# zixunh/vipe

Measured on AMD Instinct MI355X. Metric: dense-BA+flow update iters/s, 512x384 48-KF graph, higher is better.
Workload: dtype f16 (correlation, GRU; fp32 accumulate) + f32 geometry/BA (fp64 reduced system)

## Files before the change

### include/vipe_amd.h

```cpp
#ifndef VIPE_AMD_H
#define VIPE_AMD_H

#include <stdint.h>

#ifdef __cplusplus
extern "C" {
#endif

#define VIPE_F16 0
#define VIPE_F32 1
#define VIPE_F64 2
#define VIPE_U8 3

#define VIPE_OK 0
#define VIPE_EINVAL (-1)
#define VIPE_ENOSPACE (-2)
#define VIPE_EUNSUPPORTED (-3)

#define VIPE_PYRAMID_REFERENCE 0
#define VIPE_PYRAMID_BLOCKED 1

#define VIPE_CAM_PINHOLE 0
#define VIPE_CAM_MEI 1
#define VIPE_CAM_PANORAMA 2
// ... 237 lines not shown
int vipe_conv_packed_dims(int Cout, int Cin, int KH, int KW, int* cout_pad, int* cin_pad, int* k_pad);

#define VIPE_CONV_PARTIAL 6
#define VIPE_CONV_HEADS_FUSED 7
#define VIPE_CONV_ACCINIT_F32 0x100
int vipe_conv2d_fused(const void* d_x0, int x0_ctot, int x0_coff, const void* d_x1, int x1_ctot, int x1_coff,
                      int split, const void* d_w_packed, const float* d_bias, const float* d_extra, int extra_stride,
                      int extra_off, void* d_y, int y_ctot, int y_coff, void* d_y2, int y2_ctot, int y2_coff,
                      const void* d_net, int net_ctot, int net_coff, const void* d_z, float* d_fout,
                      const void* d_accinit, int ai_ctot, int ai_coff, int B, int H, int W, int Cin, int Cout, int KH,
                      int KW, int act, int mode, void* stream);

int vipe_heads_fused_ok(int H, int W);
int vipe_heads_border_floats(int E, int H, int W, int64_t* n_floats);
int vipe_heads_finish(float* d_dw, const float* d_border, const float* d_bias, int E, int H, int W, void* stream);

typedef struct {
  const void *corr0_w, *corr2_w, *flow0_w, *flow2_w, *gw_w, *zr_w, *q_w, *zr_s_w, *q_s_w, *heads0_w, *heads2_w, *agg2_w, *eta_w;
  const void *zr_n_w, *zr_x_w;
  const float *corr0_b, *corr2_b, *flow0_b, *flow2_b, *gw_b, *zr_b, *q_b, *heads0_b, *heads2_b, *agg2_b, *eta_b;
  const float* glo_wT;
  const float* glo_b;
  const void *agg1_w, *heads_dw_w;
  const float *agg1_b, *heads_dw_b;
  const void* heads2_frag;
} vipe_update_weights;
typedef struct {
  int E, H, W, n_src;
  const void* levels[4];
  const float* coords;
// ... 4 lines not shown
  const void* net;
  void* net_out;
  void* xbuf;
  const void* pgate;
  void *c1, *f1, *zb, *rnet;
  void* hbuf;
  float* dw;
  float *glo, *extra;
  const int *order, *rowptr;
  void *agg, *a2;
  float* eta;
  void* side_stream;
  float* pzr;
  int gate_state;
  float* hborder;
} vipe_update_buffers;
int vipe_update_operator(const vipe_update_weights* weights, const vipe_update_buffers* buffers, void* stream);

int vipe_update_gate_state(const vipe_update_weights* weights, const vipe_update_buffers* buffers, const void* d_net,
                           int parts, void* stream);
typedef struct {
  const vipe_update_weights* weights;
  const vipe_update_buffers* buffers;
  const void* net;
  const int* bounds;
  int n_bounds;
} vipe_gate_state_job;
int vipe_update_gate_state_piece(void* user, int piece, int n_pieces, void* stream);

int vipe_glo_context(const float* d_glo_sum, const float* d_wT, const float* d_bias, float* d_extra, int E, int hw,
// ... 93 lines not shown
```

### vipe_amd/csrc/common.cuh

```cuda
#pragma once
#include <hip/hip_runtime.h>
#include <hip/hip_fp16.h>
#include <stdint.h>

#include <atomic>
#include <mutex>

#include "../../include/vipe_amd.h"

#define VIPE_EXPORT extern "C" __attribute__((visibility("default")))

#define VIPE_CHECK_ARG(cond) \
  do {                       \
    if (!(cond)) return VIPE_EINVAL; \
  } while (0)

static inline int vipe_launch_status() {
  hipError_t e = hipGetLastError();
  return e == hipSuccess ? VIPE_OK : (int)e;
}

template <typename F>
static inline void vipe_once_per_device(std::atomic<uint64_t>& done, F&& fn) {
  int d = 0;
  (void)hipGetDevice(&d);
  const uint64_t bit = 1ull << (d & 63);
  if (done.load(std::memory_order_acquire) & bit) return;
  static std::mutex mu;
  std::lock_guard<std::mutex> lock(mu);
  if (done.load(std::memory_order_relaxed) & bit) return;
  fn();
  done.fetch_or(bit, std::memory_order_release);
}

static inline hipStream_t as_stream(void* s) { return (hipStream_t)s; }

constexpr int WAVE = 64;

template <typename T>
__device__ __forceinline__ T wave_sum(T v) {
#pragma unroll
  for (int o = 32; o > 0; o >>= 1) v += __shfl_xor(v, o, WAVE);
  return v;
}

__device__ __forceinline__ float wave_sum_to_lane63(float v) {
#define VIPE_DPP_ADD(ctrl, rmask)                                                                          \
  v += __builtin_bit_cast(float, __builtin_amdgcn_update_dpp(0, __builtin_bit_cast(int, v), ctrl, rmask, 0xf, true))
  VIPE_DPP_ADD(0xB1, 0xf);
  VIPE_DPP_ADD(0x4E, 0xf);
  VIPE_DPP_ADD(0x141, 0xf);
// ... 22 lines not shown
```

### vipe_amd/csrc/conv_mfma.hip

```cpp
#include <stdlib.h>

#include <type_traits>

#include "common.cuh"
#include "conv_call.cuh"

namespace {

typedef _Float16 half8 __attribute__((ext_vector_type(8)));
typedef _Float16 half4 __attribute__((ext_vector_type(4)));
typedef float float16v __attribute__((ext_vector_type(16)));
typedef float float4v __attribute__((ext_vector_type(4)));

struct ConvArgs {
  const half_t* x0; int x0_ctot, x0_coff;
  const half_t* x1; int x1_ctot, x1_coff;
  int split;
  const half_t* w;
  const float* bias;
  const float* extra;
  int extra_stride, extra_off;
  half_t* y; int y_ctot, y_coff;
  int B, H, W, Cin, Cin_pad, Cout, Cout_pad, KH, KW, nsteps;
  int act, epi;
// ... 1144 lines not shown
  VIPE_CHECK_ARG(d_w_oihw && d_w_packed);
  VIPE_CHECK_ARG(src_dtype == VIPE_F16 || src_dtype == VIPE_F32);
  int cp, cinp, kp;
  if (vipe_conv_packed_dims(Cout, Cin, KH, KW, &cp, &cinp, &kp) != VIPE_OK) return VIPE_EINVAL;
  VIPE_CHECK_ARG(Cin == 4 || Cin % 8 == 0);
  const int64_t total = (int64_t)kp * cp;
  pack_weights_kernel<<<(int)std::min<int64_t>((total + 255) / 256, 4096), 256, 0, as_stream(stream)>>>(
      d_w_oihw, (half_t*)d_w_packed, Cout, Cin, KH, KW, cp, cinp, kp, src_dtype == VIPE_F32, Cin == 4);
  return vipe_launch_status();
}

}

namespace {

__global__ __launch_bounds__(256) void heads_finish_kernel(float* __restrict__ dw, const float* __restrict__ border,
                                                           const float* __restrict__ bias, int64_t M, int H, int W) {
  const int64_t m = (int64_t)blockIdx.x * 256 + threadIdx.x;
  if (m >= M) return;
  const int x = (int)(m % W), y = (int)((m / W) % H), e = (int)(m / ((int64_t)W * H));
  const int xsegs = W / HALO_TW, ysegs = H / HALO_TH;
  const int ty = y / HALO_TH, tx = x / HALO_TW, py = y % HALO_TH, px = x % HALO_TW;
  const int tile = (e * ysegs + ty) * xsegs + tx;
  float4 s = reinterpret_cast<const float4*>(dw)[m];
  auto add = [&](int t, int bi) {
    const float4 v = reinterpret_cast<const float4*>(border)[(int64_t)t * HB_N + bi];
    s.x += v.x; s.y += v.y; s.z += v.z; s.w += v.w;
  };
  const bool up = py == 0 && ty > 0, down = py == HALO_TH - 1 && ty < ysegs - 1;
  const bool left = px == 0 && tx > 0, right = px == HALO_TW - 1 && tx < xsegs - 1;
  if (up) add(tile - xsegs, hb_index(HALO_TH, px));
  if (down) add(tile + xsegs, hb_index(-1, px));
  if (left) add(tile - 1, hb_index(py, HALO_TW));
  if (right) add(tile + 1, hb_index(py, -1));
  if (up && left) add(tile - xsegs - 1, hb_index(HALO_TH, HALO_TW));
  if (up && right) add(tile - xsegs + 1, hb_index(HALO_TH, -1));
  if (down && left) add(tile + xsegs - 1, hb_index(-1, HALO_TW));
  if (down && right) add(tile + xsegs + 1, hb_index(-1, -1));
  const float4 b = *reinterpret_cast<const float4*>(bias);
  const float v0 = s.x + b.x, v1 = s.y + b.y, v2 = s.z + b.z, v3 = s.w + b.w;
  reinterpret_cast<float4*>(dw)[m] = make_float4((float)(half_t)v0, (float)(half_t)v1, (float)(half_t)act_apply(v2, VIPE_ACT_SIGMOID),
                                                 (float)(half_t)act_apply(v3, VIPE_ACT_SIGMOID));
}

template <typename K>
void allow_lds(K kernel, std::atomic<uint64_t>& seen, size_t bytes) {
  vipe_once_per_device(seen, [&] { (void)hipFuncSetAttribute((const void*)kernel, hipFuncAttributeMaxDynamicSharedMemorySize, (int)bytes); });
}
constexpr size_t MAX_LDS = 160 * 1024;

bool flat_geometry(ConvArgs& a, int pad) {
  a.f_wp = a.W + pad;
  a.f_hwp = a.H * a.f_wp;
  a.f_tiles = (a.f_hwp + 255) / 256;
  a.f_magic = (unsigned)(((1ull << 32) + (unsigned)a.f_wp - 1) / (unsigned)a.f_wp);
  const int rows = 256 + 2 * a.f_wp + 2;
  a.f_pieces = (rows + 15) / 16;
// ... 209 lines not shown
VIPE_EXPORT int vipe_heads_border_floats(int E, int H, int W, int64_t* n) {
  VIPE_CHECK_ARG(n && E >= 0 && H > 0 && W > 0 && H % HALO_TH == 0 && W % HALO_TW == 0);
  *n = (int64_t)E * (H / HALO_TH) * (W / HALO_TW) * HB_N * 4;
  return VIPE_OK;
}

VIPE_EXPORT int vipe_heads_finish(float* d_dw, const float* d_border, const float* d_bias, int E, int H, int W, void* stream) {
  VIPE_CHECK_ARG(E >= 0 && H > 0 && W > 0 && H % HALO_TH == 0 && W % HALO_TW == 0);
  if (E == 0) return VIPE_OK;
  VIPE_CHECK_ARG(d_dw && d_border && d_bias);
  const int64_t M = (int64_t)E * H * W;
  heads_finish_kernel<<<(unsigned)((M + 255) / 256), 256, 0, as_stream(stream)>>>(d_dw, d_border, d_bias, M, H, W);
  return vipe_launch_status();
}

}
```

### vipe_amd/csrc/corr_lookup.hip

```cpp
#include <algorithm>
#include <type_traits>

#include "common.cuh"
#include "corr_layout.cuh"

namespace {

template <typename T>
struct Acc;

template <>
struct Acc<half_t> {
  using reg = float;
  static __device__ __forceinline__ reg load(const half_t* p) { return (float)*p; }
  static __device__ __forceinline__ reg weight(float w) {
    asm volatile("" : "+v"(w));
    return (float)(half_t)w;
  }
  static __device__ __forceinline__ reg madd(reg acc, reg s, reg w) {
    float prod = (float)(half_t)(s * w);
    return (float)(half_t)(acc + prod);
  }
  static __device__ __forceinline__ half_t store(reg v) { return (half_t)v; }
};
// ... 517 lines not shown
VIPE_EXPORT int vipe_corr_pyramid_lookup(const void* const* h_levels, const float* d_coords, void* d_out, int B,
                                         int h1, int w1, int h2, int w2, int num_levels, int radius, int dtype,
                                         void* stream) {
  return pyramid_lookup_impl(h_levels, d_coords, d_out, B, h1, w1, h2, w2, num_levels, radius, dtype, 0, stream);
}

VIPE_EXPORT int vipe_corr_pyramid_lookup_nhwc(const void* const* h_levels, const float* d_coords, void* d_out, int B,
                                              int h1, int w1, int h2, int w2, int num_levels, int radius, int dtype,
                                              int channel_stride, void* stream) {
  const int rd = 2 * radius + 1;
  VIPE_CHECK_ARG(channel_stride >= num_levels * rd * rd);
  return pyramid_lookup_impl(h_levels, d_coords, d_out, B, h1, w1, h2, w2, num_levels, radius, dtype, channel_stride,
                             stream);
}

static int device_compute_units() {
  static std::atomic<int> cus[64];
  int d = 0;
  (void)hipGetDevice(&d);
  int n = cus[d & 63].load(std::memory_order_relaxed);
  if (n > 0) return n;
  if (hipDeviceGetAttribute(&n, hipDeviceAttributeMultiprocessorCount, d) != hipSuccess || n <= 0) return 0;
  cus[d & 63].store(n, std::memory_order_relaxed);
  return n;
}

VIPE_EXPORT int vipe_corr_lookup_conv1x1(const void* const* h_levels, const float* d_coords, const void* d_w_packed,
                                         const float* d_bias, void* d_out, int out_ctot, int out_coff, int B, int h1,
                                         int w1, int h2, int w2, int Cout, int act, const int* d_slots, int layout,
                                         void* stream) {
  return vipe_corr_lookup_conv1x1_ex(h_levels, d_coords, d_w_packed, d_bias, d_out, out_ctot, out_coff, B, h1, w1, h2, w2,
                                     Cout, act, d_slots, layout, stream, 0, 0);
}

VIPE_EXPORT int vipe_corr_lookup_conv1x1_ex(const void* const* h_levels, const float* d_coords, const void* d_w_packed,
                                            const float* d_bias, void* d_out, int out_ctot, int out_coff, int B, int h1,
                                            int w1, int h2, int w2, int Cout, int act, const int* d_slots, int layout,
                                            void* stream, int max_workgroups, int share_cu) {
  VIPE_CHECK_ARG(B >= 0 && h1 > 0 && w1 > 0 && h2 > 0 && w2 > 0 && max_workgroups >= 0);
  if (B == 0) return VIPE_OK;
  VIPE_CHECK_ARG(h_levels && d_coords && d_w_packed && d_bias && d_out);
  VIPE_CHECK_ARG(act == VIPE_ACT_NONE || act == VIPE_ACT_RELU);
  VIPE_CHECK_ARG(out_ctot % 8 == 0 && out_coff % 8 == 0 && out_coff + Cout <= out_ctot);
  VIPE_CHECK_ARG(layout == VIPE_PYRAMID_REFERENCE || layout == VIPE_PYRAMID_BLOCKED);
  if (Cout != 128 || (h2 >> 3) < 1 || (w2 >> 3) < 1) return VIPE_EUNSUPPORTED;
  if (layout == VIPE_PYRAMID_REFERENCE && ((w2 >> 3) & 7) != 0) return VIPE_EUNSUPPORTED;
  if (layout == VIPE_PYRAMID_BLOCKED) VIPE_CHECK_ARG(h1 == h2 && w1 == w2);
  LevelPtrs lv;
  for (int i = 0; i < 4; ++i) {
    VIPE_CHECK_ARG(h_levels[i]);
    lv.p[i] = h_levels[i];
  }
  const int64_t ngroups = (int64_t)B * ((h1 * w1 + LKC_PX - 1) / LKC_PX);
  VIPE_CHECK_ARG(ngroups < (1 << 30));
  const int cus = device_compute_units();
  if (cus <= 0) return VIPE_EINVAL;
  int64_t blocks = std::min<int64_t>(ngroups, share_cu ? cus : 2 * cus);
  if (max_workgroups > 0) blocks = std::min<int64_t>(blocks, max_workgroups);
  const size_t lds = share_cu ? LKC_LDS_SHARED_CU : LKC_LDS;
  auto launch = [&](auto blk) {
    auto* kernel = corr_lookup_conv_kernel<decltype(blk)::value>;
    static std::atomic<uint64_t> seen{0};
    vipe_once_per_device(seen, [&] { (void)hipFuncSetAttribute((const void*)kernel, hipFuncAttributeMaxDynamicSharedMemorySize, LKC_LDS_SHARED_CU); });
    kernel<<<(int)blocks, LKC_THREADS, lds, as_stream(stream)>>>(lv, d_coords, (const half_t*)d_w_packed, d_bias, (half_t*)d_out,
                                                                 out_ctot, out_coff, h1, w1, h2, w2, B, 128, act, d_slots);
  };
  if (layout == VIPE_PYRAMID_BLOCKED) launch(std::true_type{});
  else launch(std::false_type{});
  return vipe_launch_status();
}
// ... 1 lines not shown
```

### vipe_amd/csrc/misc.hip

```cpp
#include "common.cuh"

VIPE_EXPORT const char* vipe_amd_version(void) { return "vipe_amd 0.1 (gfx950, hipcc)"; }
VIPE_EXPORT int vipe_amd_abi_version(void) { return 4; }
```

### vipe_amd/csrc/update_op.hip

```cpp
#include "common.cuh"
#include "conv_call.cuh"

namespace {

__global__ __launch_bounds__(384) void glo_gemm_kernel(const float* __restrict__ glo, const float* __restrict__ wT ,
                                                       const float* __restrict__ b, float* __restrict__ extra, float inv_hw) {
  __shared__ float g[128];
  const int e = blockIdx.x, t = threadIdx.x;
  if (t < 128) g[t] = glo[(int64_t)e * 128 + t] * inv_hw;
  __syncthreads();
  float acc = b[t];
#pragma unroll 8
  for (int k = 0; k < 128; ++k) acc = __builtin_fmaf(g[k], wT[k * 384 + t], acc);
  extra[(int64_t)e * 384 + t] = acc;
}

__global__ __launch_bounds__(256) void update_finish_kernel(const float* __restrict__ coords1, const float* __restrict__ dw,
                                                            const unsigned char* __restrict__ mask, float* __restrict__ target,
                                                            float* __restrict__ weight, const float* __restrict__ eta,
                                                            const int64_t* __restrict__ du, float* __restrict__ damping,
                                                            int64_t n_px, int64_t n_eta, int P) {
  const int64_t i = (int64_t)blockIdx.x * 256 + threadIdx.x;
  if (i < n_px) {
    const float2 c = reinterpret_cast<const float2*>(coords1)[i];
// ... 104 lines not shown
  auto agg_chain = [&](hipStream_t st) -> int {
    if (b->n_src <= 0) return VIPE_OK;
    VIPE_CHECK_ARG(b->order && b->rowptr && b->agg && b->a2 && b->eta);
    const Grid gs = {b->n_src, H, W};
    RUN(vipe_segment_mean_nhwc_f16(b->hbuf, 384, 256, b->order, b->rowptr, b->agg, b->n_src, (int64_t)H * W, 128, st));
    RUN(relu_conv(gs, {b->agg, 128, 0}, 128, wt->agg2_w, wt->agg2_b, 128, 3, {b->a2, 128, 0}, st));
    ConvCall c = conv(gs, {b->a2, 128, 0}, 128, wt->eta_w, wt->eta_b, 1, 3);
    c.epi = EPI_ETA; c.fout = b->eta;
    return vipe_conv_run(c, st);
  };
  auto heads2 = [&](hipStream_t st) -> int {
    ConvCall c = conv(g, {b->hbuf, 384, 0}, 256, wt->heads2_w, wt->heads2_b, 4, 3);
    c.epi = EPI_HEADS; c.fout = b->dw;
    return vipe_conv_run(c, st);
  };
  if (by_consumer && two_tails) {
    RUN(heads0(wt->agg1_w, wt->agg1_b, 256, 128));
    VIPE_CHECK_ARG(fork(2));
    RUN(agg_chain(side));
    if (wt->heads2_frag && b->hborder && vipe_heads_fused_ok(H, W)) {
      ConvCall c = conv(g, {b->net_out, 128, 0}, 128, wt->heads_dw_w, wt->heads_dw_b, 256, 3);
      c.act = VIPE_ACT_RELU; c.epi = EPI_HEADS_FUSED; c.heads2_frag = wt->heads2_frag; c.border = b->hborder; c.fout = b->dw;
      RUN(vipe_conv_run(c, s));
      RUN(vipe_heads_finish(b->dw, b->hborder, wt->heads2_b, E, H, W, stream));
    } else {
      RUN(heads0(wt->heads_dw_w, wt->heads_dw_b, 0, 256));
      RUN(heads2(s));
    }
  } else {
    RUN(heads0(wt->heads0_w, wt->heads0_b, 0, 384));
    if (two_tails) VIPE_CHECK_ARG(fork(2));
    RUN(heads2(two_tails ? s2 : s));
    RUN(agg_chain(s));
  }
  if (two_tails) VIPE_CHECK_ARG(join(3));
  return vipe_launch_status();
}

VIPE_EXPORT int vipe_update_gate_state(const vipe_update_weights* wt, const vipe_update_buffers* b, const void* d_net,
                                       int parts, void* stream) {
  VIPE_CHECK_ARG(wt && b && b->E >= 0 && b->H > 0 && b->W > 0 && parts >= 1 && parts <= 3);
  if (b->E == 0) return VIPE_OK;
  VIPE_CHECK_ARG(d_net && (!(parts & 1) || (b->glo && b->extra)) && (!(parts & 2) || (b->pgate && b->pzr && wt->zr_n_w)));
  if (parts & 1) RUN(global_context(wt, b, d_net, as_stream(stream)));
  if (parts & 2) {
    ConvCall c = conv({b->E, b->H, b->W}, {d_net, 128, 0}, 128, wt->zr_n_w, wt->zr_b, 256, 3);
    c.epi = EPI_PARTIAL; c.accinit = {b->pgate, 384, 0};
    c.fout = b->pzr; c.y = {nullptr, 256, 0};
    RUN(vipe_conv_run(c, as_stream(stream)));
  }
// ... 49 lines not shown
```

### vipe_amd/ext/slam_ext.py

```python

import ctypes

import torch

from .._lib import CAMERA_CODE, BAParams, check, check_gpu_contig, lib, ptr, require, stream_ptr

_WS = {}


def _workspace(device, nbytes):
    key = (device.type, device.index)
    ws = _WS.get(key)
    if ws is None or ws.numel() < nbytes:
        ws = torch.empty(int(nbytes * 1.25) + 1024, dtype=torch.uint8, device=device)
        _WS[key] = ws
    return ws


def _i64(t):
    require(t.dtype == torch.int64, "index tensors must be int64")
    return t


def reproject(poses, disps, intrinsics, rig, pi, qi, pj, qj, di, camera="pinhole", intr_factor=8.0, want_valid=True):
# ... 38 lines not shown
        coords = torch.empty((M, ht, wd, 2), dtype=torch.float32, device=poses.device)
        motn = torch.empty((M, ht, wd, 4), dtype=torch.float16, device=poses.device)
    check(lib().vipe_reproject_motion_nhwc(ptr(poses), ptr(disps), ptr(intrinsics), ptr(rig), ptr(_i64(pi)),
                                           ptr(_i64(qi)), ptr(_i64(pj)), ptr(_i64(qj)), ptr(_i64(di)), ptr(target),
                                           ptr(coords), ptr(motn), M, ht, wd, rig.shape[0], CAMERA_CODE[camera],
                                           float(intr_factor), stream_ptr(poses)), "reproject_motion_nhwc")
    return coords, motn


def update_finish(coords1, dw, mask, target, weight, eta, du, damping):
    E, ht, wd, _ = coords1.shape
    n_src = 0 if eta is None else int(eta.shape[0])
    require(target.is_contiguous() and weight.is_contiguous() and target.numel() == E * ht * wd * 2, "target / weight: contiguous [1,E,h,w,2]")
    check(lib().vipe_update_finish(ptr(coords1), ptr(dw), ptr(mask), ptr(target), ptr(weight), ptr(eta), ptr(du), ptr(damping),
                                   E, n_src, ht, wd, stream_ptr(coords1)), "update_finish")


def _camera_code(camera):
    if camera not in CAMERA_CODE:
        raise ValueError(f"unknown camera {camera!r} (one of {sorted(CAMERA_CODE)})")
    return CAMERA_CODE[camera]


def _check_camera_options(camera, optimize_intrinsics):
    _camera_code(camera)
    if camera == "panorama" and optimize_intrinsics:
        raise ValueError("the panorama camera has no intrinsics: optimize_intrinsics cannot be combined with it")


BA_OPT_ONE_CHAIN, BA_OPT_GENERAL_ACCUMULATE = 1, 2
# ... 219 lines not shown
```

### vipe_amd/slam/factor_graph.py

```python

import ctypes
import dataclasses
import os

import numpy as np
import torch

from .._lib import check, check_gpu_contig, lib, parse_struct, require, stream_ptr, upload, upload_many
from ..ext import slam_ext
from .edge_index import NAMES, EdgeIndex, as_host
from .networks import AltCorrBlock, CorrBlock, CorrPool

WORK = {"edge_updates": 0, "pyramids_built": 0}
BACKEND_VOLUME_GB = 160


def warm_volume_pool(device, gigabytes=None):
    if torch.device(device).type != "cuda":
        return 0
    want = float(gigabytes if gigabytes is not None else os.environ.get("VIPE_AMD_BACKEND_VOLUME_GB", BACKEND_VOLUME_GB)) * 2**30
    free, _ = torch.cuda.mem_get_info(device)
    n = int(min(want, 0.85 * free))
    if n <= 0:
        return 0
# ... 155 lines not shown


def _index_property(name):
    def put(self, tensor):
        self._index.assign(name, tensor)
        if name != "age":
            self._edges_changed()

    return property(lambda self: self._index.device(name), put)


class FactorGraph:
    upsample = False
    upsample_from_row = None
    _last_ba = None

    def __init__(self, update_module, buffer, device, max_factors=48, incremental=True, cross_view=False):
        self.update_op = update_module
        self.buffer = buffer
        self.device = device
        self.max_factors = max_factors
        self.incremental = incremental
        self.cross_view = cross_view and buffer.n_views > 1
        ht, wd = buffer.height // 8, buffer.width // 8
        self.ht, self.wd = ht, wd
        self.damping = 1e-6 * torch.ones_like(buffer.flattened_disps)
        self.target = torch.zeros([1, 0, ht, wd, 2], device=device, dtype=torch.float)
        self.weight = torch.zeros([1, 0, ht, wd, 2], device=device, dtype=torch.float)
        self.corr, self.net_n, self.xbuf = None, None, None
        self.pgate = None
# ... 217 lines not shown
            self._plan_serial += 1
            if self.cross_view or self.buffer.n_views > 1:
                from .update_engine import segment_csr
                du, dix = torch.unique(di, return_inverse=True)
                n_src = int(du.numel())
                csr = segment_csr(dix, n_src)
            else:
                du_h, dix_h = np.unique(ii_h, return_inverse=True)
                du, dix = upload_many([du_h, dix_h], self.device)
                n_src = int(du_h.shape[0])
                csr = tuple(upload_many(host_csr(dix_h, n_src), self.device, torch.int32))
            self._plan = dict(pi=pi, qi=qi, di=di, pj=pj, qj=qj, du=du, dix=dix, n_src=n_src, csr=csr,
                              t0=int(max(1, ii_h.min() + 1)), t1=int(max(ii_h.max(), jj_h.max()) + 1), base=int(min(ii_h.min(), jj_h.min())))
        return self._plan

    def _inactive_room(self, k):
        n = self.target_inac.shape[1]
        cap = self._inac_cap
        if cap is None or cap[0].shape[1] < n + k or cap[0].data_ptr() != self.target_inac.data_ptr():
            size = max(2 * (n + k), 256)
            cap = tuple(torch.empty((1, size) + tuple(x.shape[2:]), dtype=x.dtype, device=x.device)
                        for x in (self.target_inac, self.weight_inac))
            cap[0][:, :n] = self.target_inac
            cap[1][:, :n] = self.weight_inac
            self._inac_cap = cap
        self.target_inac, self.weight_inac = cap[0][:, :n + k], cap[1][:, :n + k]
        return cap[0], cap[1], n

    def _upsample_disps(self, mask, du, own=None):
        from ..ext import droid_net_ext
# ... 44 lines not shown
        t1 = P["t1"] if t1 is None else t1
        buf = self.buffer
        E_act = int(P["pi"].shape[0])
        WORK["edge_updates"] += E_act
        if "io" not in P:
            P["io"] = (torch.empty((E_act, self.ht, self.wd, 2), dtype=torch.float32, device=self.device),
                       torch.empty((E_act, self.ht, self.wd, 4), dtype=torch.float16, device=self.device))
            P["mask"] = buf.masks[P["pi"], P["qi"]].contiguous()
        self._contiguous_targets()
        coords1, motn = slam_ext.reproject_motion_nhwc(buf.poses, buf.flattened_disps, buf.intrinsics, buf.rig,
                                                       P["pi"], P["qi"], P["pj"], P["qj"], P["di"],
                                                       self.target[0], camera=buf.camera_type, out=P["io"])
        eng = self.update_op.engine(self.device)
        corr = self.corr.lookup_deferred(coords1)
        up = {"want_upmask": True} if self.upsample else {}
        self.net_n, dw, eta, upmask = eng.forward_nhwc(self.net_n, self.xbuf, corr, motn, ix=P["dix"], n_src=P["n_src"],
                                                       net_out=self._net_spare(), csr=P["csr"], pgate=self.pgate,
                                                       gate_state=self._gate_state, **up)
        self._gate_state = None
        overlap = self.pgate is not None and E_act >= self.gate_overlap_min_edges
        ba_overlap = None
        if overlap:
            main = torch.cuda.current_stream(self.device)
            if self._side is None:
                self._side = torch.cuda.Stream(device=self.device)
            self._side.wait_stream(main)
            n_staged = max(1, int(round(self.gate_overlap_share * E_act)))
            if self.gate_overlap_mode == "gated":
                with torch.cuda.stream(self._side):
                    eng.hidden_gate_state(self.net_n, self.pgate, parts=1)
                fr = self.gate_overlap_fractions if len(self.gate_overlap_fractions) == itrs else None
                gate_state, ov = eng.gate_state_job(self.net_n, self.pgate, fractions=fr, n_staged=n_staged)
                ba_overlap = ov(self._side)
            else:
                with torch.cuda.stream(self._side):
                    gate_state = eng.hidden_gate_state(self.net_n, self.pgate, n_staged=n_staged)
        slam_ext.update_finish(coords1, dw, P["mask"], self.target, self.weight, eta, P["du"], self.damping)
        if use_inactive:
            key = ("inac", t0)
            if key not in P:
                h = self._index.host
                sel_h = np.flatnonzero((h["ii_inac"] >= t0 - 3) & (h["jj_inac"] >= t0 - 3))
                ii, jj, sel_exp = upload_many([np.concatenate([h["ii_inac"][sel_h], h["ii"]]),
                                               np.concatenate([h["jj_inac"][sel_h], h["jj"]]),
                                               per_view(sel_h, buf.n_views)], self.device)
                base = int(min(h["ii"].min(), h["jj"].min(), *(h[k][sel_h].min() for k in ("ii_inac", "jj_inac") if sel_h.size)))
                plan = self._shift_plan(buf.expand_edge_multiview(ii, jj)[:5], base)
                n_sel = int(sel_exp.shape[0])
                comb = tuple(torch.empty((1, n_sel + E_act) + tuple(x.shape[2:]), dtype=x.dtype, device=x.device)
                             for x in (self.target, self.weight))
                comb[0][:, :n_sel] = self.target_inac.index_select(1, sel_exp)
                comb[1][:, :n_sel] = self.weight_inac.index_select(1, sel_exp)
# ... 118 lines not shown
```

### vipe_amd/slam/update_engine.py

```python

import ctypes
import os

import torch

from .._lib import check, lib, parse_struct, ptr, stream_ptr

UpdateWeights = parse_struct("vipe_update_weights")
UpdateBuffers = parse_struct("vipe_update_buffers")
GateStateJob = parse_struct("vipe_gate_state_job")

ACT = {"none": 0, "relu": 1, "sigmoid": 2, "tanh": 3}
EPI = {"plain": 0, "glo": 1, "zr": 2, "q": 3, "heads": 4, "eta": 5, "partial": 6, "heads_fused": 7}
ACCINIT_F32 = 0x100
CORR_CH = 200


class _Packed:

    def __init__(self, w_oihw, bias, device):
        w = w_oihw.detach().to(device=device, dtype=torch.float16).contiguous()
        self.cout, self.cin, self.kh, self.kw = w.shape
        cp, cinp, kp = ctypes.c_int(), ctypes.c_int(), ctypes.c_int()
        check(lib().vipe_conv_packed_dims(self.cout, self.cin, self.kh, self.kw, ctypes.addressof(cp),
# ... 27 lines not shown
    order = torch.argsort(ix, stable=True).to(torch.int32).contiguous()
    counts = torch.bincount(ix, minlength=n_src)
    rowptr = torch.zeros(n_src + 1, dtype=torch.int32, device=ix.device)
    rowptr[1:] = torch.cumsum(counts, 0).to(torch.int32)
    return order, rowptr


class UpdateEngine:
    def __init__(self, module, device):
        self.device = device
        self.m = module
        self._bufs = {}
        self._op_side = None
        self.op_side_min_edges = int(os.environ.get("VIPE_AMD_OP_SIDE_MIN_EDGES", "64"))
        self._gate_gen = 0
        self._pack_all()

    def _pack_all(self):
        m, d = self.m, self.device
        f16 = torch.float16

        def wb(conv):
            return conv.weight.detach().to(d, f16), conv.bias.detach().to(d, torch.float32)

        w, b = wb(m.corr_encoder[0])
        w = torch.cat([w, torch.zeros(128, CORR_CH - 196, 1, 1, device=d, dtype=f16)], 1)
        self.corr0 = _Packed(w, b, d)
        self.corr2 = _Packed(*wb(m.corr_encoder[2]), d)
        self.flow0 = _Packed(*wb(m.flow_encoder[0]), d)
        self.flow2 = _Packed(*wb(m.flow_encoder[2]), d)
# ... 138 lines not shown

    def _hborder(self, E, H, W):
        n = ctypes.c_int64()
        check(lib().vipe_heads_border_floats(E, H, W, ctypes.addressof(n)), "heads_border_floats")
        return self._buf("hborder", (n.value,), torch.float32)

    def _buf(self, name, shape, dtype=torch.float16):
        t = self._bufs.get(name)
        if t is None or tuple(t.shape) != tuple(shape) or t.dtype != dtype:
            t = torch.empty(shape, dtype=dtype, device=self.device)
            self._bufs[name] = t
        return t

    @torch.no_grad()
    def forward_nhwc(self, net, xbuf, corr, motn, ix=None, n_src=None, net_out=None, want_upmask=False, csr=None,
                     pgate=None, native=True, gate_state=None):
        E, H, W, _ = net.shape
        if not self.gate_state_matches(gate_state, net, pgate):
            gate_state = None
        if gate_state is None:
            self._gate_gen += 1
        c1 = self._buf("c1", (E, H, W, 128))
        f1 = self._buf("f1", (E, H, W, 128))
        zb = self._buf("z", (E, H, W, 128))
        rnet = self._buf("rnet", (E, H, W, 128))
        hbuf = self._buf("h", (E, H, W, 384))
        dw = self._buf("dw", (E, H, W, 4), torch.float32)
        glo = self._buf("glo", (E, 128), torch.float32)
        if net_out is None:
            net_out = torch.empty_like(net)
        if native:
            return self._forward_native(net, xbuf, corr, motn, ix, n_src, net_out, want_upmask, csr, pgate,
                                        (c1, f1, zb, rnet, hbuf, dw, glo), gate_state)
        if isinstance(corr, tuple):
            from ..ext import droid_net_ext
            droid_net_ext.corr_lookup_conv1x1(corr[1], corr[2], self.corr0.packed, self.corr0.bias, c1, act="relu",
                                              slots=corr[3] if len(corr) > 3 else None,
                                              grid=corr[4] if len(corr) > 4 else None)
        else:
            self._conv(self.corr0, corr, 0, E, H, W, y=c1, act="relu", cin=CORR_CH)
        self._conv(self.corr2, c1, 0, E, H, W, y=xbuf, y_coff=128, act="relu")
        self._conv(self.flow0, motn, 0, E, H, W, y=f1, act="relu")
        self._conv(self.flow2, f1, 0, E, H, W, y=xbuf, y_coff=256, act="relu")
        extra = self._buf("extra", (E, 384), torch.float32)
        if gate_state is None:
            glo.zero_()
            self._conv(self.gw, net, 0, E, H, W, mode="glo", net=net, fout=glo)
            check(lib().vipe_glo_context(ptr(glo), ptr(self.glo_w), ptr(self.glo_b), ptr(extra), E, H * W, stream_ptr(glo)),
# ... 43 lines not shown
                      "heads_finish")
            else:
                self._conv(self.heads_dw, net_out, 0, E, H, W, y=hbuf, act="relu")
                self._conv(self.heads2, hbuf, 0, E, H, W, mode="heads", fout=dw, cin=256)
        else:
            self._conv(self.heads0, net_out, 0, E, H, W, y=hbuf, act="relu")
            self._conv(self.heads2, hbuf, 0, E, H, W, mode="heads", fout=dw, cin=256)
            if ix is not None:
                a2, eta = agg_chain()
        if ix is not None and want_upmask:
            upmask = torch.empty((n_src, H, W, 576), dtype=torch.float16, device=self.device)
            self._conv(self.upmask, a2, 0, n_src, H, W, y=upmask)
        return net_out, dw, eta, upmask

    def _forward_native(self, net, xbuf, corr, motn, ix, n_src, net_out, want_upmask, csr, pgate, scratch,
                        gate_state=None):
        c1, f1, zb, rnet, hbuf, dw, glo = scratch
        E, H, W, _ = net.shape
        extra = self._buf("extra", (E, 384), torch.float32)
        eta = agg = a2 = order = rowptr = None
        if ix is not None:
            if n_src is None:
                n_src = int(ix.max().item()) + 1 if ix.numel() else 0
            if csr is None:
                csr = segment_csr(ix, n_src)
            order, rowptr = csr
            agg = self._buf("agg", (n_src, H, W, 128))
            a2 = self._buf("a2", (n_src, H, W, 128))
            eta = self._buf("eta", (n_src, H, W), torch.float32)
        lookup = isinstance(corr, tuple)
        hborder = self._hborder(E, H, W) if self.fused_heads(H, W) else None
        tensors = (net, net_out, xbuf, motn, pgate, c1, f1, zb, rnet, hbuf, dw, glo, extra, order, rowptr, agg, a2, eta,
                   hborder) + \
            ((tuple(corr[1]) + (corr[2],) + ((corr[3],) if len(corr) > 3 and corr[3] is not None else ())) if lookup else (corr,))
        pzr = gate_state["pzr"] if gate_state is not None else None
        two_streams = E >= self.op_side_min_edges
        if two_streams and self._op_side is None:
            self._op_side = torch.cuda.Stream(device=self.device)
        key = tuple(0 if t is None else t.data_ptr() for t in tensors) + (E, H, W, n_src or 0, two_streams,
                                                                         0 if pzr is None else pzr.data_ptr(),
                                                                         0 if pzr is None else int(gate_state["n_staged"]))
        b = self._bdesc.get(key)
        if b is None:
            if len(self._bdesc) > 16:
                self._bdesc.clear()
            b = UpdateBuffers()
            b.E, b.H, b.W, b.n_src = E, H, W, int(n_src or 0) if ix is not None else 0
            if lookup:
                lv = corr[1]
                for i in range(4):
                    b.levels[i] = lv[i].data_ptr()
                b.coords = corr[2].data_ptr()
                b.slots = corr[3].data_ptr() if len(corr) > 3 and corr[3] is not None else None
                if len(corr) > 4 and corr[4] is not None:
                    b.h2, b.w2 = int(corr[4][0]), int(corr[4][1])
                else:
                    b.h2, b.w2 = int(lv[2].shape[3]) << 2, int(lv[2].shape[4]) << 2
                b.pyramid_layout = 1 if lv[0].dim() == 7 else 0
            else:
                b.corr = corr.data_ptr()
            for name, t in dict(motn=motn, net=net, net_out=net_out, xbuf=xbuf, pgate=pgate, c1=c1, f1=f1, zb=zb, rnet=rnet,
                                hbuf=hbuf, dw=dw, glo=glo, extra=extra, order=order, rowptr=rowptr, agg=agg, a2=a2,
                                eta=eta, hborder=hborder).items():
                setattr(b, name, None if t is None else t.data_ptr())
            if pzr is not None:
                b.pzr, b.gate_state = pzr.data_ptr(), int(gate_state["n_staged"])
            if two_streams:
                b.side_stream = self._op_side.cuda_stream
            self._bdesc[key] = b
        check(lib().vipe_update_operator(ctypes.addressof(self._wdesc), ctypes.addressof(b), stream_ptr(net)),
              "update_operator")
        upmask = None
        if want_upmask and ix is not None:
            upmask = torch.empty((n_src, H, W, 576), dtype=torch.float16, device=self.device)
            self._conv(self.upmask, a2, 0, n_src, H, W, y=upmask)
        return net_out, dw, eta, upmask

    @torch.no_grad()
    def forward(self, net, inp, corr, flow=None, ix=None, skip_upmask=False, n_src=None):
        batch, num, ch, ht, wd = net.shape
        E = batch * num
        dev = net.device
        f16 = torch.float16
        net_n = net.reshape(E, 128, ht, wd).to(f16).permute(0, 2, 3, 1).contiguous()
        xbuf = torch.empty((E, ht, wd, 320), dtype=f16, device=dev)
        xbuf[..., 0:128] = inp.reshape(E, 128, ht, wd).permute(0, 2, 3, 1)
        corr_n = torch.zeros((E, ht, wd, CORR_CH), dtype=f16, device=dev)
        corr_n[..., :196] = corr.reshape(E, 196, ht, wd).permute(0, 2, 3, 1)
        if flow is None:
            motn_n = torch.zeros((E, ht, wd, 4), dtype=f16, device=dev)
        else:
# ... 15 lines not shown
```

Before: 274.9.

## Fuse heads-finish into update-finish kernel and add optional tail context/gate split

Adds a kernel that performs the heads border reduction, bias and sigmoid together with the target/weight/damping writes of update_finish, so the separate heads_finish launch and its extra pass over dw are skipped when enabled (default on). It also adds an opt-in path that computes the next global context on the side stream at the operator's tail, and an opt-in round-aware choice of how many edges are staged for the gate overlap. The fused path moves the heads finishing off the operator's stream and into the later finish call, which changes when dw becomes final.

```diff
diff --git a/include/vipe_amd.h b/include/vipe_amd.h
--- a/include/vipe_amd.h
+++ b/include/vipe_amd.h
@@ -275,6 +275,12 @@
 int vipe_heads_fused_ok(int H, int W);
 int vipe_heads_border_floats(int E, int H, int W, int64_t* n_floats);
 int vipe_heads_finish(float* d_dw, const float* d_border, const float* d_bias, int E, int H, int W, void* stream);
+int vipe_update_finish_heads(const float* d_coords1, float* d_dw, const float* d_border, const float* d_bias,
+                             const unsigned char* d_mask, float* d_target, float* d_weight, const float* d_eta,
+                             const int64_t* d_du, float* d_damping, int E, int n_src, int H, int W, void* stream);
+
+int vipe_gate_split_edges_slots(int E, int H, int W, double share, int slots, int* n_staged);
+int vipe_gate_split_edges(int E, int H, int W, double share, int* n_staged);
 
 typedef struct {
   const void *corr0_w, *corr2_w, *flow0_w, *flow2_w, *gw_w, *zr_w, *q_w, *zr_s_w, *q_s_w, *heads0_w, *heads2_w, *agg2_w, *eta_w;
@@ -309,6 +315,8 @@
   float* pzr;
   int gate_state;
   float* hborder;
+  int next_context;
+  int skip_heads_finish;
 } vipe_update_buffers;
 int vipe_update_operator(const vipe_update_weights* weights, const vipe_update_buffers* buffers, void* stream);
 
diff --git a/vipe_amd/csrc/common.cuh b/vipe_amd/csrc/common.cuh
--- a/vipe_amd/csrc/common.cuh
+++ b/vipe_amd/csrc/common.cuh
@@ -35,6 +35,17 @@
 
 static inline hipStream_t as_stream(void* s) { return (hipStream_t)s; }
 
+static inline int vipe_device_compute_units() {
+  static std::atomic<int> cus[64];
+  int d = 0;
+  (void)hipGetDevice(&d);
+  int n = cus[d & 63].load(std::memory_order_relaxed);
+  if (n > 0) return n;
+  if (hipDeviceGetAttribute(&n, hipDeviceAttributeMultiprocessorCount, d) != hipSuccess || n <= 0) return 0;
+  cus[d & 63].store(n, std::memory_order_relaxed);
+  return n;
+}
+
 constexpr int WAVE = 64;
 
 template <typename T>
diff --git a/vipe_amd/csrc/conv_mfma.hip b/vipe_amd/csrc/conv_mfma.hip
--- a/vipe_amd/csrc/conv_mfma.hip
+++ b/vipe_amd/csrc/conv_mfma.hip
@@ -1182,10 +1182,8 @@
 
 namespace {
 
-__global__ __launch_bounds__(256) void heads_finish_kernel(float* __restrict__ dw, const float* __restrict__ border,
-                                                           const float* __restrict__ bias, int64_t M, int H, int W) {
-  const int64_t m = (int64_t)blockIdx.x * 256 + threadIdx.x;
-  if (m >= M) return;
+__device__ __forceinline__ float4 heads_finish_px(const float* __restrict__ dw, const float* __restrict__ border,
+                                                  const float* __restrict__ bias, int64_t m, int H, int W) {
   const int x = (int)(m % W), y = (int)((m / W) % H), e = (int)(m / ((int64_t)W * H));
   const int xsegs = W / HALO_TW, ysegs = H / HALO_TH;
   const int ty = y / HALO_TH, tx = x / HALO_TW, py = y % HALO_TH, px = x % HALO_TW;
@@ -1207,8 +1205,34 @@
   if (down && right) add(tile + xsegs + 1, hb_index(-1, -1));
   const float4 b = *reinterpret_cast<const float4*>(bias);
   const float v0 = s.x + b.x, v1 = s.y + b.y, v2 = s.z + b.z, v3 = s.w + b.w;
-  reinterpret_cast<float4*>(dw)[m] = make_float4((float)(half_t)v0, (float)(half_t)v1, (float)(half_t)act_apply(v2, VIPE_ACT_SIGMOID),
-                                                 (float)(half_t)act_apply(v3, VIPE_ACT_SIGMOID));
+  return make_float4((float)(half_t)v0, (float)(half_t)v1, (float)(half_t)act_apply(v2, VIPE_ACT_SIGMOID),
+                     (float)(half_t)act_apply(v3, VIPE_ACT_SIGMOID));
+}
+
+__global__ __launch_bounds__(256) void heads_finish_kernel(float* __restrict__ dw, const float* __restrict__ border,
+                                                           const float* __restrict__ bias, int64_t M, int H, int W) {
+  const int64_t m = (int64_t)blockIdx.x * 256 + threadIdx.x;
+  if (m >= M) return;
+  reinterpret_cast<float4*>(dw)[m] = heads_finish_px(dw, border, bias, m, H, W);
+}
+
+__global__ __launch_bounds__(256) void finish_heads_kernel(const float* __restrict__ coords1, float* __restrict__ dw,
+                                                           const float* __restrict__ border, const float* __restrict__ bias,
+                                                           const unsigned char* __restrict__ mask, float* __restrict__ target,
+                                                           float* __restrict__ weight, const float* __restrict__ eta,
+                                                           const int64_t* __restrict__ du, float* __restrict__ damping,
+                                                           int64_t n_px, int64_t n_eta, int H, int W) {
+  const int64_t i = (int64_t)blockIdx.x * 256 + threadIdx.x;
+  const int P = H * W;
+  if (i < n_px) {
+    const float4 d = heads_finish_px(dw, border, bias, i, H, W);
+    const float2 c = reinterpret_cast<const float2*>(coords1)[i];
+    const bool m = mask && mask[i];
+    reinterpret_cast<float4*>(dw)[i] = d;
+    reinterpret_cast<float2*>(target)[i] = make_float2(c.x + d.x, c.y + d.y);
+    reinterpret_cast<float2*>(weight)[i] = m ? make_float2(0.f, 0.f) : make_float2(d.z, d.w);
+  }
+  if (i < n_eta) damping[du[i / P] * P + i % P] = eta[i];
 }
 
 template <typename K>
@@ -1448,4 +1472,45 @@
   return vipe_launch_status();
 }
 
-}
+VIPE_EXPORT int vipe_update_finish_heads(const float* d_coords1, float* d_dw, const float* d_border, const float* d_bias,
+                                         const unsigned char* d_mask, float* d_target, float* d_weight, const float* d_eta,
+                                         const int64_t* d_du, float* d_damping, int E, int n_src, int H, int W, void* stream) {
+  VIPE_CHECK_ARG(E >= 0 && n_src >= 0 && H > 0 && W > 0 && H % HALO_TH == 0 && W % HALO_TW == 0);
+  if (E == 0) return VIPE_OK;
+  VIPE_CHECK_ARG(d_coords1 && d_dw && d_border && d_bias && d_target && d_weight && (n_src == 0 || (d_eta && d_du && d_damping)));
+  const int64_t n_px = (int64_t)E * H * W, n_eta = (int64_t)n_src * H * W;
+  const int64_t n = n_px > n_eta ? n_px : n_eta;
+  finish_heads_kernel<<<(unsigned)((n + 255) / 256), 256, 0, as_stream(stream)>>>(d_coords1, d_dw, d_border, d_bias, d_mask, d_target,
+                                                                                 d_weight, d_eta, d_du, d_damping, n_px, n_eta, H, W);
+  return vipe_launch_status();
+}
+
+VIPE_EXPORT int vipe_gate_split_edges_slots(int E, int H, int W, double share, int slots, int* n_staged) {
+  VIPE_CHECK_ARG(n_staged && E >= 1 && H > 0 && W > 0 && share > 0.0 && share <= 1.0 && slots >= 0);
+  const double want = share * E;
+  const int own = (int)std::min<double>(E, std::max(1.0, nearbyint(want)));
+  *n_staged = own;
+  ConvArgs a = {};
+  a.H = H; a.W = W;
+  int64_t tiles;
+  if (W % HALO_TW == 0 && H % HALO_TH == 0) tiles = (int64_t)H * W / (HALO_TH * HALO_TW);
+  else if (flat_geometry(a, 1)) tiles = a.f_tiles;
+  else return VIPE_OK;
+  if (slots == 0) return VIPE_OK;
+  const int64_t per_edge = tiles * 2;
+  auto rounds = [&](int n) { return (n * per_edge + slots - 1) / slots; };
+  auto total = [&](int n) { return rounds(n) + rounds(E - n); };
+  auto whole = [&](int n) { return n * per_edge % slots == 0; };
+  int best = own;
+  for (int n = 1; n <= E; ++n) {
+    if (fabs(n - want) > 0.15 * E || total(n) >= total(own)) continue;
+    const bool better = best == own || total(n) < total(best) ||
+                        (total(n) == total(best) && (whole(n) > whole(best) ||
+                                                     (whole(n) == whole(best) && fabs(n - want) < fabs(best - want))));
+    if (better) best = n;
+  }
+  *n_staged = best;
+  return VIPE_OK;
+}
+
+}
diff --git a/vipe_amd/csrc/corr_lookup.hip b/vipe_amd/csrc/corr_lookup.hip
--- a/vipe_amd/csrc/corr_lookup.hip
+++ b/vipe_amd/csrc/corr_lookup.hip
@@ -555,17 +555,6 @@
                              stream);
 }
 
-static int device_compute_units() {
-  static std::atomic<int> cus[64];
-  int d = 0;
-  (void)hipGetDevice(&d);
-  int n = cus[d & 63].load(std::memory_order_relaxed);
-  if (n > 0) return n;
-  if (hipDeviceGetAttribute(&n, hipDeviceAttributeMultiprocessorCount, d) != hipSuccess || n <= 0) return 0;
-  cus[d & 63].store(n, std::memory_order_relaxed);
-  return n;
-}
-
 VIPE_EXPORT int vipe_corr_lookup_conv1x1(const void* const* h_levels, const float* d_coords, const void* d_w_packed,
                                          const float* d_bias, void* d_out, int out_ctot, int out_coff, int B, int h1,
                                          int w1, int h2, int w2, int Cout, int act, const int* d_slots, int layout,
@@ -594,7 +583,7 @@
   }
   const int64_t ngroups = (int64_t)B * ((h1 * w1 + LKC_PX - 1) / LKC_PX);
   VIPE_CHECK_ARG(ngroups < (1 << 30));
-  const int cus = device_compute_units();
+  const int cus = vipe_device_compute_units();
   if (cus <= 0) return VIPE_EINVAL;
   int64_t blocks = std::min<int64_t>(ngroups, share_cu ? cus : 2 * cus);
   if (max_workgroups > 0) blocks = std::min<int64_t>(blocks, max_workgroups);
diff --git a/vipe_amd/csrc/misc.hip b/vipe_amd/csrc/misc.hip
--- a/vipe_amd/csrc/misc.hip
+++ b/vipe_amd/csrc/misc.hip
@@ -2,3 +2,7 @@
 
 VIPE_EXPORT const char* vipe_amd_version(void) { return "vipe_amd 0.1 (gfx950, hipcc)"; }
 VIPE_EXPORT int vipe_amd_abi_version(void) { return 4; }
+
+VIPE_EXPORT int vipe_gate_split_edges(int E, int H, int W, double share, int* n_staged) {
+  return vipe_gate_split_edges_slots(E, H, W, share, 2 * vipe_device_compute_units(), n_staged);
+}
diff --git a/vipe_amd/csrc/update_op.hip b/vipe_amd/csrc/update_op.hip
--- a/vipe_amd/csrc/update_op.hip
+++ b/vipe_amd/csrc/update_op.hip
@@ -142,26 +142,31 @@
     c.epi = EPI_HEADS; c.fout = b->dw;
     return vipe_conv_run(c, st);
   };
+  const bool ctx_side = s2 && b->next_context;
+  if (b->next_context) VIPE_CHECK_ARG(b->glo && b->extra && b->net_out);
   if (by_consumer && two_tails) {
     RUN(heads0(wt->agg1_w, wt->agg1_b, 256, 128));
     VIPE_CHECK_ARG(fork(2));
     RUN(agg_chain(side));
+    if (b->next_context) RUN(global_context(wt, b, b->net_out, side));
     if (wt->heads2_frag && b->hborder && vipe_heads_fused_ok(H, W)) {
       ConvCall c = conv(g, {b->net_out, 128, 0}, 128, wt->heads_dw_w, wt->heads_dw_b, 256, 3);
       c.act = VIPE_ACT_RELU; c.epi = EPI_HEADS_FUSED; c.heads2_frag = wt->heads2_frag; c.border = b->hborder; c.fout = b->dw;
       RUN(vipe_conv_run(c, s));
-      RUN(vipe_heads_finish(b->dw, b->hborder, wt->heads2_b, E, H, W, stream));
+      if (!b->skip_heads_finish) RUN(vipe_heads_finish(b->dw, b->hborder, wt->heads2_b, E, H, W, stream));
     } else {
       RUN(heads0(wt->heads_dw_w, wt->heads_dw_b, 0, 256));
       RUN(heads2(s));
     }
   } else {
     RUN(heads0(wt->heads0_w, wt->heads0_b, 0, 384));
-    if (two_tails) VIPE_CHECK_ARG(fork(2));
+    if (two_tails || ctx_side) VIPE_CHECK_ARG(fork(2));
     RUN(heads2(two_tails ? s2 : s));
+    if (ctx_side) RUN(global_context(wt, b, b->net_out, side));
     RUN(agg_chain(s));
-  }
-  if (two_tails) VIPE_CHECK_ARG(join(3));
+    if (b->next_context && !s2) RUN(global_context(wt, b, b->net_out, s));
+  }
+  if (two_tails || ctx_side) VIPE_CHECK_ARG(join(3));
   return vipe_launch_status();
 }
 
diff --git a/vipe_amd/ext/slam_ext.py b/vipe_amd/ext/slam_ext.py
--- a/vipe_amd/ext/slam_ext.py
+++ b/vipe_amd/ext/slam_ext.py
@@ -76,6 +76,15 @@
     require(target.is_contiguous() and weight.is_contiguous() and target.numel() == E * ht * wd * 2, "target / weight: contiguous [1,E,h,w,2]")
     check(lib().vipe_update_finish(ptr(coords1), ptr(dw), ptr(mask), ptr(target), ptr(weight), ptr(eta), ptr(du), ptr(damping),
                                    E, n_src, ht, wd, stream_ptr(coords1)), "update_finish")
+
+
+def update_finish_heads(coords1, dw, border, bias, mask, target, weight, eta, du, damping):
+    E, ht, wd, _ = coords1.shape
+    n_src = 0 if eta is None else int(eta.shape[0])
+    require(target.is_contiguous() and weight.is_contiguous() and target.numel() == E * ht * wd * 2, "target / weight: contiguous [1,E,h,w,2]")
+    check(lib().vipe_update_finish_heads(ptr(coords1), ptr(dw), ptr(border), ptr(bias), ptr(mask), ptr(target), ptr(weight),
+                                         ptr(eta), ptr(du), ptr(damping), E, n_src, ht, wd, stream_ptr(coords1)),
+          "update_finish_heads")
 
 
 def _camera_code(camera):
diff --git a/vipe_amd/slam/factor_graph.py b/vipe_amd/slam/factor_graph.py
--- a/vipe_amd/slam/factor_graph.py
+++ b/vipe_amd/slam/factor_graph.py
@@ -193,6 +193,9 @@
     upsample = False
     upsample_from_row = None
     _last_ba = None
+    tail_context = os.environ.get("VIPE_AMD_TAIL_CONTEXT", "0") != "0"
+    gate_round_split = os.environ.get("VIPE_AMD_GATE_ROUND_SPLIT", "0") != "0"
+    fused_finish = os.environ.get("VIPE_AMD_FUSED_FINISH", "1") != "0"
 
     def __init__(self, update_module, buffer, device, max_factors=48, incremental=True, cross_view=False):
         self.update_op = update_module
@@ -440,6 +443,16 @@
                               t0=int(max(1, ii_h.min() + 1)), t1=int(max(ii_h.max(), jj_h.max()) + 1), base=int(min(ii_h.min(), jj_h.min())))
         return self._plan
 
+    def _n_staged(self, P, E_act):
+        key = ("n_staged", self.gate_overlap_share, self.gate_round_split)
+        if key not in P:
+            n = ctypes.c_int(max(1, int(round(self.gate_overlap_share * E_act))))
+            if self.gate_round_split:
+                check(lib().vipe_gate_split_edges(E_act, self.ht, self.wd, float(self.gate_overlap_share), ctypes.addressof(n)),
+                      "gate_split_edges")
+            P[key] = int(n.value)
+        return P[key]
+
     def _inactive_room(self, k):
         n = self.target_inac.shape[1]
         cap = self._inac_cap
@@ -514,28 +527,31 @@
         eng = self.update_op.engine(self.device)
         corr = self.corr.lookup_deferred(coords1)
         up = {"want_upmask": True} if self.upsample else {}
+        overlap = self.pgate is not None and E_act >= self.gate_overlap_min_edges
+        tail_context = overlap and self.gate_overlap_mode == "gated" and self.tail_context and E_act >= eng.op_side_min_edges
         self.net_n, dw, eta, upmask = eng.forward_nhwc(self.net_n, self.xbuf, corr, motn, ix=P["dix"], n_src=P["n_src"],
                                                        net_out=self._net_spare(), csr=P["csr"], pgate=self.pgate,
-                                                       gate_state=self._gate_state, **up)
+                                                       gate_state=self._gate_state, next_context=tail_context,
+                                                       finish_heads=not self.fused_finish, **up)[:4]
         self._gate_state = None
-        overlap = self.pgate is not None and E_act >= self.gate_overlap_min_edges
         ba_overlap = None
         if overlap:
             main = torch.cuda.current_stream(self.device)
             if self._side is None:
                 self._side = torch.cuda.Stream(device=self.device)
             self._side.wait_stream(main)
-            n_staged = max(1, int(round(self.gate_overlap_share * E_act)))
+            n_staged = self._n_staged(P, E_act)
             if self.gate_overlap_mode == "gated":
-                with torch.cuda.stream(self._side):
-                    eng.hidden_gate_state(self.net_n, self.pgate, parts=1)
+                if not tail_context:
+                    with torch.cuda.stream(self._side):
+                        eng.hidden_gate_state(self.net_n, self.pgate, parts=1)
                 fr = self.gate_overlap_fractions if len(self.gate_overlap_fractions) == itrs else None
                 gate_state, ov = eng.gate_state_job(self.net_n, self.pgate, fractions=fr, n_staged=n_staged)
                 ba_overlap = ov(self._side)
             else:
                 with torch.cuda.stream(self._side):
                     gate_state = eng.hidden_gate_state(self.net_n, self.pgate, n_staged=n_staged)
-        slam_ext.update_finish(coords1, dw, P["mask"], self.target, self.weight, eta, P["du"], self.damping)
+        eng.finish_update(coords1, dw, P["mask"], self.target, self.weight, eta, P["du"], self.damping)
         if use_inactive:
             key = ("inac", t0)
             if key not in P:
diff --git a/vipe_amd/slam/update_engine.py b/vipe_amd/slam/update_engine.py
--- a/vipe_amd/slam/update_engine.py
+++ b/vipe_amd/slam/update_engine.py
@@ -65,6 +65,7 @@
         self._op_side = None
         self.op_side_min_edges = int(os.environ.get("VIPE_AMD_OP_SIDE_MIN_EDGES", "64"))
         self._gate_gen = 0
+        self.heads_unfinished = None
         self._pack_all()
 
     def _pack_all(self):
@@ -233,11 +234,12 @@
 
     @torch.no_grad()
     def forward_nhwc(self, net, xbuf, corr, motn, ix=None, n_src=None, net_out=None, want_upmask=False, csr=None,
-                     pgate=None, native=True, gate_state=None):
+                     pgate=None, native=True, gate_state=None, next_context=False, finish_heads=True):
         E, H, W, _ = net.shape
+        assert native or (not next_context and finish_heads)
         if not self.gate_state_matches(gate_state, net, pgate):
             gate_state = None
-        if gate_state is None:
+        if gate_state is None or next_context:
             self._gate_gen += 1
         c1 = self._buf("c1", (E, H, W, 128))
         f1 = self._buf("f1", (E, H, W, 128))
@@ -250,7 +252,7 @@
             net_out = torch.empty_like(net)
         if native:
             return self._forward_native(net, xbuf, corr, motn, ix, n_src, net_out, want_upmask, csr, pgate,
-                                        (c1, f1, zb, rnet, hbuf, dw, glo), gate_state)
+                                        (c1, f1, zb, rnet, hbuf, dw, glo), gate_state, next_context, finish_heads)
         if isinstance(corr, tuple):
             from ..ext import droid_net_ext
             droid_net_ext.corr_lookup_conv1x1(corr[1], corr[2], self.corr0.packed, self.corr0.bias, c1, act="relu",
@@ -324,7 +326,7 @@
         return net_out, dw, eta, upmask
 
     def _forward_native(self, net, xbuf, corr, motn, ix, n_src, net_out, want_upmask, csr, pgate, scratch,
-                        gate_state=None):
+                        gate_state=None, next_context=False, finish_heads=True):
         c1, f1, zb, rnet, hbuf, dw, glo = scratch
         E, H, W, _ = net.shape
         extra = self._buf("extra", (E, 384), torch.float32)
@@ -347,9 +349,12 @@
         two_streams = E >= self.op_side_min_edges
         if two_streams and self._op_side is None:
             self._op_side = torch.cuda.Stream(device=self.device)
+        skip_finish = not finish_heads and hborder is not None and two_streams and ix is not None and n_src > 0
+        self.heads_unfinished = (dw, hborder) if skip_finish else None
         key = tuple(0 if t is None else t.data_ptr() for t in tensors) + (E, H, W, n_src or 0, two_streams,
                                                                          0 if pzr is None else pzr.data_ptr(),
-                                                                         0 if pzr is None else int(gate_state["n_staged"]))
+                                                                         0 if pzr is None else int(gate_state["n_staged"]),
+                                                                         bool(next_context), skip_finish)
         b = self._bdesc.get(key)
         if b is None:
             if len(self._bdesc) > 16:
@@ -377,6 +382,7 @@
                 b.pzr, b.gate_state = pzr.data_ptr(), int(gate_state["n_staged"])
             if two_streams:
                 b.side_stream = self._op_side.cuda_stream
+            b.next_context, b.skip_heads_finish = int(bool(next_context)), int(skip_finish)
             self._bdesc[key] = b
         check(lib().vipe_update_operator(ctypes.addressof(self._wdesc), ctypes.addressof(b), stream_ptr(net)),
               "update_operator")
@@ -384,7 +390,15 @@
         if want_upmask and ix is not None:
             upmask = torch.empty((n_src, H, W, 576), dtype=torch.float16, device=self.device)
             self._conv(self.upmask, a2, 0, n_src, H, W, y=upmask)
-        return net_out, dw, eta, upmask
+        return (net_out, dw, eta, upmask, extra) if next_context else (net_out, dw, eta, upmask)
+
+    def finish_update(self, coords1, dw, mask, target, weight, eta, du, damping):
+        from ..ext import slam_ext
+        pending, self.heads_unfinished = self.heads_unfinished, None
+        if pending is None:
+            return slam_ext.update_finish(coords1, dw, mask, target, weight, eta, du, damping)
+        assert pending[0].data_ptr() == dw.data_ptr()
+        slam_ext.update_finish_heads(coords1, dw, pending[1], self.heads2.bias, mask, target, weight, eta, du, damping)
 
     @torch.no_grad()
     def forward(self, net, inp, corr, flow=None, ix=None, skip_upmask=False, n_src=None):
```

New measurement: 273.9. Within noise of the previous version (-0.4%).
